# jhidalgocarrio/slam-localization

Measured on AMD Instinct MI355X. Metric: filter predict+update steps/sec, higher is better.
Workload: dtype f64

## Files before the change

slam-localization_amd/csrc/slk_kernels.hpp:

```cpp
#pragma once
#include <hip/hip_runtime.h>

#include "../../include/slk.h"
#include "slk_math.hpp"

namespace slk {

typedef double d4 __attribute__((ext_vector_type(4)));
typedef float f4 __attribute__((ext_vector_type(4)));
typedef __bf16 b8 __attribute__((ext_vector_type(8)));

constexpr int KP = 8;
constexpr int STEP_WGS = 4;
constexpr int MAXM = 32;
constexpr int PRED_SCRATCH = 1536;

struct Lay { int kind, k, nfk, nfkl, N, Nq, nso3; };

struct KArgs {
    int B;
    Lay lay;
    double *mean; double *P; int *status; unsigned *outliers;
    int do_predict, pm; const double *u; int u_stride; const double *Q; int q_stride; const double *Yext;
    int do_update, mm; const double *mp; int mp_stride; const double *z; int m;
// ... 299 lines not shown
        }
    int fail = -1;
    CholCols<NTHREADS, SD, 0>::run(a, Lp, n, colbuf, ti, tj, active, fail);
    __syncthreads();
    return (fail >= n) ? -1 : fail;
}

__host__ __device__ constexpr int tile_idx(int I, int J) { return I * (I + 1) / 2 + J; }

__device__ __forceinline__ void wave_sync() { asm volatile("s_waitcnt lgkmcnt(0)" ::: "memory"); }

template <int NT> struct CholM {
    static constexpr int NTL = NT * (NT + 1) / 2;
    static constexpr int LDC = 16 * NT + 2;
    static constexpr int COLBUF = 4 * LDC;
};

template <int NT, class InitFn>
__device__ __forceinline__ void cholm_load(d4 (&acc)[CholM<NT>::NTL], int n, int lane, InitFn init)
{
    const int c = lane & 15, g = lane >> 4;
#pragma unroll
    for (int I = 0; I < NT; ++I)
#pragma unroll
        for (int J = 0; J <= I; ++J)
#pragma unroll
            for (int r = 0; r < 4; ++r) {
                int row = 16 * I + g + 4 * r, col = 16 * J + c;
                double v;
                if (row < n && col < n) v = (row >= col) ? init(row, col) : init(col, row);
                else v = (row == col) ? 1.0 : 0.0;
                acc[tile_idx(I, J)][r] = -v;
            }
}

template <int NT, class InitFn>
__device__ __forceinline__ void cholm_load_t(d4 (&acc)[CholM<NT>::NTL], int n, int lane, InitFn init)
{
    const int c = lane & 15, g = lane >> 4;
#pragma unroll
    for (int J = 0; J < NT; ++J)
#pragma unroll
        for (int I = J; I < NT; ++I)
#pragma unroll
            for (int r = 0; r < 4; ++r) {
                int row = 16 * I + c, col = 16 * J + g + 4 * r;
                double v;
                if (row < n && col < n) v = (row >= col) ? init(row, col) : init(col, row);
                else v = (row == col) ? 1.0 : 0.0;
                acc[tile_idx(I, J)][r] = -v;
            }
}

template <int NT, class XFn, class YFn>
__device__ __forceinline__ void cholm_downdate(d4 (&acc)[CholM<NT>::NTL], int n, int kk, int lane, XFn xel, YFn yel)
{
    const int c = lane & 15, g = lane >> 4;
    for (int ks = 0; ks * 4 < kk; ++ks) {
        const int cc = 4 * ks + g;
        double af[NT], bf[NT];
#pragma unroll
        for (int I = 0; I < NT; ++I) {
            int rho = 16 * I + c;
            bool ok = cc < kk && rho < n;
            af[I] = ok ? xel(rho, cc) : 0.0;
            bf[I] = ok ? yel(rho, cc) : 0.0;
        }
#pragma unroll
        for (int I = 0; I < NT; ++I)
#pragma unroll
            for (int J = 0; J <= I; ++J)
                acc[tile_idx(I, J)] = __builtin_amdgcn_mfma_f64_16x16x4f64(af[I], bf[J], acc[tile_idx(I, J)], 0, 0, 0);
    }
}

template <int NT, int JK>
struct CholMCols {
    __device__ __forceinline__ static void run(d4 (&acc)[CholM<NT>::NTL], double *Lp, int n, double *colbuf, int lane, int &fail)
    {
        if constexpr (JK < NT) {
            constexpr int LDC = CholM<NT>::LDC;
            const int c = lane & 15, g = lane >> 4;
            if (fail < 0) {
                for (int c0 = 0; c0 < 16; c0 += 4) {
                    const int k0 = 16 * JK + c0;
                    if (k0 >= n) break;
                    if (c >= c0 && c < c0 + 4) {
                        double *dst = colbuf + (c - c0) * LDC + g;
#pragma unroll
                        for (int I = JK; I < NT; ++I)
#pragma unroll
                            for (int r = 0; r < 4; ++r) dst[16 * I + 4 * r] = acc[tile_idx(I, JK)][r];
                    }
                    wave_sync();
                    const double *pb = colbuf + k0;
                    const double p00 = -pb[0], p10 = -pb[1], p20 = -pb[2], p30 = -pb[3];
                    const double p11 = -pb[LDC + 1], p21 = -pb[LDC + 2], p31 = -pb[LDC + 3];
                    const double p22 = -pb[2 * LDC + 2], p32 = -pb[2 * LDC + 3], p33 = -pb[3 * LDC + 3];
                    double v[NT][4];
#pragma unroll
                    for (int I = JK; I < NT; ++I)
#pragma unroll
                        for (int b = 0; b < 4; ++b) v[I][b] = -colbuf[b * LDC + 16 * I + c];
                    wave_sync();
                    double s0, r0, s1, r1, s2, r2, s3, r3;
                    if (!(p00 > 0.0)) { fail = k0; break; }
// ... 5 lines not shown
                    const double l21 = fma(-l20, l10, p21) * r1, l31 = fma(-l30, l10, p31) * r1;
                    const double d2 = fma(-l21, l21, fma(-l20, l20, p22));
                    if (!(d2 > 0.0)) { fail = k0 + 2; break; }
                    rsqrt_pivot(d2, s2, r2);
                    const double l32 = fma(-l31, l21, fma(-l30, l20, p32)) * r2;
                    const double d3 = fma(-l32, l32, fma(-l31, l31, fma(-l30, l30, p33)));
                    if (!(d3 > 0.0)) { fail = k0 + 3; break; }
                    rsqrt_pivot(d3, s3, r3);
                    const int kap = k0 + g;
                    const double sg = (g == 0) ? s0 : (g == 1) ? s1 : (g == 2) ? s2 : s3;
                    double frag[NT];
#pragma unroll
                    for (int I = JK; I < NT; ++I) {
                        const double vi0 = v[I][0], vi1 = v[I][1], vi2 = v[I][2], vi3 = v[I][3];
                        const double x0 = vi0 * r0;
                        const double x1 = fma(-x0, l10, vi1) * r1;
                        const double x2 = fma(-x1, l21, fma(-x0, l20, vi2)) * r2;
                        const double x3 = fma(-x2, l32, fma(-x1, l31, fma(-x0, l30, vi3))) * r3;
                        double f = (g == 0) ? x0 : (g == 1) ? x1 : (g == 2) ? x2 : x3;
                        const int rho = 16 * I + c;
                        if (rho == kap) f = sg;
                        if (rho < kap) f = 0.0;
                        frag[I] = f;
                        if (rho >= kap && rho < n && kap < n) Lp[pk(n, rho, kap)] = f;
                    }
#pragma unroll
                    for (int J = JK; J < NT; ++J)
#pragma unroll
                        for (int I = J; I < NT; ++I)
                            acc[tile_idx(I, J)] = __builtin_amdgcn_mfma_f64_16x16x4f64(frag[I], frag[J], acc[tile_idx(I, J)], 0, 0, 0);
                }
            }
            CholMCols<NT, JK + 1>::run(acc, Lp, n, colbuf, lane, fail);
        }
    }
};

template <int NT>
__device__ __forceinline__ int cholm_factor(d4 (&acc)[CholM<NT>::NTL], double *Lp, int n, double *colbuf, int lane)
{
    int fail = -1;
    __builtin_amdgcn_s_setprio(3);
    CholMCols<NT, 0>::run(acc, Lp, n, colbuf, lane, fail);
    wave_sync();
    __builtin_amdgcn_s_setprio(0);
    return fail;
}

__device__ __forceinline__ double readlane_f64(double x, int l)
{
    return __hiloint2double(__builtin_amdgcn_readlane(__double2hiint(x), l), __builtin_amdgcn_readlane(__double2loint(x), l));
}

template <int NT, int JK, int C0, int OUT = 1>
struct CholPSteps {
    __device__ __forceinline__ static void run(d4 (&acc)[CholM<NT>::NTL], double *Lp, int n, double *colbuf, int lane, bool &bad)
    {
        if constexpr (JK < NT) {
            constexpr int LDC = CholM<NT>::LDC;
            constexpr int k0 = 16 * JK + C0;
            if (k0 < n) {
                const int c = lane & 15, g = lane >> 4;
                const int row = (NT == 4) ? lane : min(lane, 16 * NT - 1);
                auto live = [&](int p) { return OUT != 2 || k0 + p < n; };
                const bool last = OUT == 2 && k0 + 4 >= n;
#pragma unroll
                for (int I = JK; I < NT; ++I) colbuf[g * LDC + 16 * I + c] = acc[tile_idx(I, JK)][C0 / 4];
                wave_sync();
                double l[4];
#pragma unroll
                for (int p = 0; p < 4; ++p) l[p] = live(p) ? -colbuf[p * LDC + row] : 0.0;
#pragma unroll
                for (int p = 0; p < 4; ++p) {
                    if (!live(p)) continue;
                    const double d = readlane_f64(l[p], k0 + p);
                    {
                        int nb = !(d > 0.0);
                        asm volatile("" : "+v"(nb));
                        bad |= (nb != 0);
                    }
                    double sq, rs;
                    rsqrt_pivot(d, sq, rs);
                    (void)sq;
                    l[p] *= rs;
#pragma unroll
                    for (int q = p + 1; q < 4; ++q)
                        if (live(q)) l[q] = fma(-l[p], readlane_f64(l[p], k0 + q), l[q]);
                }
                if (!last) {
                    wave_sync();
                    if (NT == 4 || lane < 16 * NT) {
#pragma unroll
                        for (int p = 0; p < 4; ++p) colbuf[p * LDC + lane] = l[p];
                    }
                }
#pragma unroll
                for (int p = 0; p < 4; ++p) {
                    if constexpr (OUT == 2) {
                        if (lane >= 16 * JK && (NT == 4 || lane < 16 * NT)) {
                            const int It = lane >> 4;
                            Lp[(It * (It + 1) / 2 + JK) * 256 + (C0 + p) * 16 + (lane & 15)] = (k0 + p < n && lane >= k0 + p) ? l[p] : 0.0;
                        }
                    } else if constexpr (OUT == 1) {
                        typedef __attribute__((address_space(1))) double gdouble;
                        unsigned long long colb = reinterpret_cast<unsigned long long>(Lp + pkcol(n, k0 + p));
                        asm volatile("" : "+s"(colb));
                        gdouble *colp = reinterpret_cast<gdouble *>(colb);
                        if (k0 + p < n && lane >= k0 + p && lane < n) colp[lane] = l[p];
                    } else {
                        if (k0 + p < n && lane >= k0 + p && lane < n) Lp[pkcol(n, k0 + p) + lane] = l[p];
                    }
                }
                if (!last) {
                    constexpr int J0 = (C0 == 12) ? JK + 1 : JK;
                    wave_sync();
                    double frag[NT];
#pragma unroll
                    for (int I = J0; I < NT; ++I) frag[I] = colbuf[g * LDC + 16 * I + c];
                    wave_sync();
#pragma unroll
                    for (int J = J0; J < NT; ++J)
#pragma unroll
                        for (int I = J; I < NT; ++I)
                            acc[tile_idx(I, J)] = __builtin_amdgcn_mfma_f64_16x16x4f64(frag[J], frag[I], acc[tile_idx(I, J)], 0, 0, 0);
                }
            } else if constexpr (OUT == 2) {
                if (lane >= 16 * JK && (NT == 4 || lane < 16 * NT)) {
                    const int It = lane >> 4;
#pragma unroll
                    for (int p = 0; p < 4; ++p) Lp[(It * (It + 1) / 2 + JK) * 256 + (C0 + p) * 16 + (lane & 15)] = 0.0;
                }
            }
            CholPSteps<NT, (C0 == 12 ? JK + 1 : JK), (C0 + 4) & 15, OUT>::run(acc, Lp, n, colbuf, lane, bad);
        }
    }
};

template <int NT, int OUT = 1>
__device__ __forceinline__ int cholp_factor(d4 (&acc)[CholM<NT>::NTL], double *Lp, int n, double *colbuf, int lane)
{
    bool bad = false;
    CholPSteps<NT, 0, 0, OUT>::run(acc, Lp, n, colbuf, lane, bad);
    wave_sync();
    return bad ? 0 : -1;
}

template <int NMAX, class InitFn>
__device__ __forceinline__ int chol_rows(double *Lp, int n, int lane, InitFn init, int nst = -1)
{
    if (nst < 0) nst = n;
    static_assert(NMAX <= 32, "chol_rows keeps a row per lane in registers");
    double a[NMAX];
#pragma unroll
    for (int j = 0; j < NMAX; ++j) {
        a[j] = init(min(lane, n - 1), j < n ? j : 0);
        if ((j & 3) == 3) __builtin_amdgcn_sched_barrier(0);
    }
    bool bad = false;
#pragma unroll
    for (int j = 0; j < NMAX; ++j) {
        if (j < n) {
            const double d = readlane_f64(a[j], j);
            bad |= !(d > 0.0);
            double sq, rs;
            rsqrt_pivot(d, sq, rs);
            (void)sq;
            a[j] *= rs;
#pragma unroll
            for (int k = j + 1; k < NMAX; ++k) a[k] = fma(-a[j], readlane_f64(a[j], k), a[k]);
            __builtin_amdgcn_sched_barrier(0);
        }
    }
    if (lane < nst) {
#pragma unroll
        for (int j = 0; j < NMAX; ++j)
            if (j < nst && lane >= j) Lp[pk(nst, lane, j)] = a[j];
    }
    wave_sync();
    return bad ? 0 : -1;
}

template <int NT, class InitFn>
__device__ __forceinline__ void cholw_load(d4 (&acc)[NT], int n, int lane, int wave, InitFn init)
{
    const int c = lane & 15, g = lane >> 4;
#pragma unroll
    for (int J = 0; J < NT; ++J)
#pragma unroll
        for (int r = 0; r < 4; ++r) {
            int row = 16 * wave + g + 4 * r, col = 16 * J + c;
            double v = 0.0;
            if (J <= wave && wave < NT) {
                if (row < n && col < n) v = (row >= col) ? init(row, col) : init(col, row);
                else v = (row == col) ? 1.0 : 0.0;
            }
            acc[J][r] = -v;
        }
// ... 1043 lines not shown
                constexpr int I = TileMap<NT>::row(T), J = TileMap<NT>::col(T);
                const int c = 16 * J + (lane & 15), rc = MfmaTiles<NT, NW, 0>::rho_of(c);
#pragma unroll
                for (int r = 0; r < 4; ++r) {
                    const int rr = 16 * I + 4 * (lane >> 4) + r;
                    if (rr < N && c < N) {
                        const int r1 = MfmaTiles<NT, NW, 0>::rho_of(rr);
                        double v = (double)acc[T / NW][r];
                        if (r1 >= 0 && rc >= 0) {
                            const int hi = r1 > rc ? r1 : rc, lo = r1 > rc ? rc : r1;
                            const int ti = hi >> 4, tj = lo >> 4;
                            v += EEt[(ti * (ti + 1) / 2 + tj) * 272 + (lo & 15) * 17 + (hi & 15)];
                        }
                        gP[c + (size_t)rr * N] = v;
                        if (I != J) gP[rr + (size_t)c * N] = v;
                    }
                }
            }
            MfmaTiles32<NT, NW, T + 1>::store_plus_rot(gP, N, acc, wave, lane, EEt);
        }
    }
    __device__ __forceinline__ static void store(double *gP, int N, const f4 (&acc)[TPW], int wave, int lane, int pass)
    {
        if constexpr (T < TileMap<NT>::NTILES) {
            if ((T % NW) == wave && (T / PER_PASS) == pass) {
                constexpr int I = TileMap<NT>::row(T), J = TileMap<NT>::col(T);
                int c = 16 * J + (lane & 15);
#pragma unroll
                for (int r = 0; r < 4; ++r) {
                    int rr = 16 * I + 4 * (lane >> 4) + r;
                    if (rr < N && c < N) {
                        double v = 0.5 * (double)acc[(T % PER_PASS) / NW][r];
                        gP[c + (size_t)rr * N] = v;
                        if (I != J) gP[rr + (size_t)c * N] = v;
                    }
                }
            }
            MfmaTiles32<NT, NW, T + 1>::store(gP, N, acc, wave, lane, pass);
        }
    }
};

template <int K> __device__ __forceinline__ bool msckf_step_fast(const KArgs &a, double *smem);
template <int NT, int NTHREADS, int KST, int MST> struct HasFastStep {
    static constexpr bool value = KST >= 4 && KST <= 8 && MST == 8 && NTHREADS == 256 && NT == (12 + 6 * KST + 15) / 16;
};

template <int NT, int NTHREADS, int KST = -1, int MST = 0>
__global__ __launch_bounds__(NTHREADS, (NTHREADS >= 256 && NT >= 3 && NT <= 4 ? (MST > 0 ? STEP_WGS : 2) : ((NT >= 5 && NT <= 8) ? 2 : (NT <= 2 ? 4 : 1)))) void msckf_step_kernel(KArgs a)
{
    constexpr bool BIG = NT > 4;
    extern __shared__ __attribute__((aligned(16))) double smem[];
    if constexpr (HasFastStep<NT, NTHREADS, KST, MST>::value) {
        if (!a.do_predict && a.do_update && msckf_step_fast<KST>(a, smem)) return;
    }
    constexpr int NW = NTHREADS / 64;
    constexpr int NROWS = (NT <= 2 && KST >= 0) ? 12 + 6 * KST : 1;
    static_assert(NT > 2 || NTHREADS == 64, "states of N <= 32 run one wave per filter");
    const int bidx = blockIdx.x, tid = threadIdx.x, lane = tid & 63, wave = tid >> 6;
    Lay L = a.lay;
    L.kind = SLK_MSCKF;
    if constexpr (KST >= 0) { L.k = KST; L.N = 12 + 6 * KST; L.Nq = 13 + 7 * KST; L.nso3 = 1 + KST; }
    if constexpr (MST > 0) { a.m = MST; a.emit = 0; a.do_update = 1; if (NT <= 4) a.rebuild_prec = 0; }
    const int N = L.N, Nq = L.Nq, m = a.m, nso3 = L.nso3;
    const Carve cv = carve_step(L, m, NT, BIG, (KST >= 0 && MST > 0 && !BIG) ? 0 : a.rebuild_prec);
    const int S = cv.S, LDD = cv.LDD;
    double *Lp = BIG ? a.wsL + (size_t)bidx * pk_size(N) : smem + cv.Lp;
    double *mu = smem + cv.mu, *ref = smem + cv.ref;
    double *delta = smem + cv.delta, *md = smem + cv.md, *colbuf = smem + cv.colbuf, *pool = smem + cv.pool, *cq = smem + cv.cq;
    int *ish = reinterpret_cast<int *>(smem + cv.small);
    int *roff = ish + 48;
    double *gmean = a.mean + (size_t)bidx * Nq;
    double *gP = a.P + (size_t)bidx * N * N;
    double *omean = a.mean_out ? a.mean_out + (size_t)bidx * Nq : gmean;
    double *oP = a.P_out ? a.P_out + (size_t)bidx * N * N : gP;
    int status = 0;
    if (a.do_update && a.emit != 4 && tid == 0) a.outliers[bidx] = 0u;
    SLK_STAMP(0);

    for (int e = tid; e < Nq; e += NTHREADS) mu[e] = gmean[e];
    if (tid == 0) {
        int o = 0;
        for (int b = 0; b < nso3; ++b) { roff[b] = o; o += rot_count(L, b); }
        roff[nso3] = o;
        ish[42] = 0;
    }
    __syncthreads();
    SLK_STAMP(1);

    constexpr bool WCHOL = NT >= 3 && NT <= 4 && NW >= NT;
    bool pred12 = false;
    const double *Pn12 = smem + cv.pn12;
    if constexpr (NT <= 2) {
        if (a.do_predict) {
            double *Lblk = pool, *Pn = pool + 160, *scr = pool + 320;
            const int st = predict_phase<false>(a, bidx, tid, [&](int i, int j) { return gP[i + (size_t)j * N]; }, Lblk, mu, Pn, scr,
                                                nullptr);
            if (st < 0) return;
            status |= st;
            if (!(st & SLK_ST_LLT_FAIL)) {
                for (int e = tid; e < 144; e += NTHREADS) {
                    smem[cv.pn12 + e] = Pn[e];
                    gP[(e % 12) + (size_t)(e / 12) * N] = Pn[e];
                }
                if (tid < 13) gmean[tid] = mu[tid];
                pred12 = true;
// ... 1241 lines not shown
```

slam-localization_amd/csrc/slk_math.hpp:

```cpp
#pragma once
#include <hip/hip_runtime.h>

namespace slk {

struct Quat { double x, y, z, w; };

__device__ __forceinline__ Quat qmul(const Quat &a, const Quat &b)
{
    Quat o;
    o.w = a.w * b.w - a.x * b.x - a.y * b.y - a.z * b.z;
    o.x = a.w * b.x + a.x * b.w + a.y * b.z - a.z * b.y;
    o.y = a.w * b.y + a.y * b.w + a.z * b.x - a.x * b.z;
    o.z = a.w * b.z + a.z * b.w + a.x * b.y - a.y * b.x;
    return o;
}

__device__ __forceinline__ Quat qconj(const Quat &q) { return Quat{-q.x, -q.y, -q.z, q.w}; }

__device__ __forceinline__ void qrot(const Quat &q, double vx, double vy, double vz,
                                     double &ox, double &oy, double &oz)
{
    double ux = q.y * vz - q.z * vy, uy = q.z * vx - q.x * vz, uz = q.x * vy - q.y * vx;
    ux += ux; uy += uy; uz += uz;
    ox = vx + q.w * ux + (q.y * uz - q.z * uy);
    oy = vy + q.w * uy + (q.z * ux - q.x * uz);
    oz = vz + q.w * uz + (q.x * uy - q.y * ux);
}

struct CosSinc { double c, s; };
__device__ __forceinline__ CosSinc cos_sinc_sqrt_libm_body(double x)
{
    const double sx = sqrt(x);
    return CosSinc{cos(sx), sin(sx) / sx};
}
__device__ __forceinline__ double so3_log_scale_libm_body(double n2, double w)
{
    double nv = sqrt(n2);
    if (nv < 1e-11) nv = 1e-11;
    return 2.0 / nv * atan(nv / w);
}
__device__ __attribute__((noinline)) CosSinc cos_sinc_sqrt_libm(double x) { return cos_sinc_sqrt_libm_body(x); }
__device__ __attribute__((noinline)) double so3_log_scale_libm(double n2, double w) { return so3_log_scale_libm_body(n2, w); }

template <bool LEAF = false>
__device__ __forceinline__ void cos_sinc_sqrt(double x, double &c, double &s)
{
    if (x < 0.25) {
        const double y = -x;
        double cc = 0x1.1d8d32755f8fbp-29;
        cc = fma(cc, y, 0x1.27e40964b47d4p-22);
        cc = fma(cc, y, 0x1.a01a00fb1bc6fp-16);
        cc = fma(cc, y, 0x1.6c16c16bdd04ep-10);
        cc = fma(cc, y, 0x1.5555555555421p-5);
        cc = fma(cc, y, 0x1.fffffffffffffp-2);
        cc = fma(cc, y, 1.0);
        double ss = 0x1.ac53ce336f805p-26;
        ss = fma(ss, y, 0x1.71dd113fb7905p-19);
        ss = fma(ss, y, 0x1.a01a01061c190p-13);
        ss = fma(ss, y, 0x1.11111110ecfb3p-7);
        ss = fma(ss, y, 0x1.555555555548fp-3);
        ss = fma(ss, y, 1.0);
        c = cc;
        s = ss;
    } else {
        const CosSinc r = LEAF ? cos_sinc_sqrt_libm_body(x) : cos_sinc_sqrt_libm(x);
        c = r.c;
        s = r.s;
    }
}

template <bool LEAF = false>
__device__ __forceinline__ Quat so3_exp(double vx, double vy, double vz)
{
    double c, s;
    cos_sinc_sqrt<LEAF>(0.25 * (vx * vx + vy * vy + vz * vz), c, s);
    double m = s * 0.5;
    return Quat{m * vx, m * vy, m * vz, c};
}

__device__ __forceinline__ double rcp_refined(double a)
// ... 119 lines not shown
```

slam-localization_amd/csrc/slk_step_fast.hpp:

```cpp
#pragma once
#ifdef SLK_STAMPS
#define SLK_FSTAMP(i) do { SLK_STAMP_NR(i); if (a.stop > 0 && a.stop == (i)) return true; } while (0)
#define SLK_WSTAMP(w, i) do { if (tid == 64 * (w) && a.dbg) a.dbg[(size_t)bidx * 32 + (i)] = clock64(); } while (0)
#define SLK_FBAIL(code) do { SLK_NOTE(28, code); return false; } while (0)
#else
#define SLK_FSTAMP(i) do { } while (0)
#define SLK_WSTAMP(w, i) do { } while (0)
#define SLK_FBAIL(code) return false
#endif

namespace slk {

template <int K> struct FastShape {
    static constexpr int N = 12 + 6 * K, Nq = 13 + 7 * K, S = 2 * N + 1, NSO3 = K + 1;
    static constexpr int NT = (N + 15) / 16, NTL = NT * (NT + 1) / 2, NKS = (N + 3) / 4;
    static constexpr int NROT = 3 * NSO3;
    static constexpr int NP = 3 * K * K + 15 * K + 6;
    static constexpr int NIT = NP + NSO3;
    static constexpr int RND = (NIT + 255) / 256;
    static constexpr int oLt = 0;
    static constexpr int oMu = oLt + NTL * 256;
    static constexpr int oRef = oMu + ((Nq + 7) & ~7);
    static constexpr int oDelta = oRef + ((Nq + 7) & ~7);
    static constexpr int oMd = oDelta + 64;
// ... 150 lines not shown
        for (int i = 0; i < NV; ++i) f[i] = fma(f[i], y[i], ak);
    }
#pragma unroll
    for (int i = 0; i < NV; ++i) {
        f[i] = fma(f[i], y[i], 1.0);
        const double sv = sc[i] * f[i];
        d[i][0] = sv * q[i].x; d[i][1] = sv * q[i].y; d[i][2] = sv * q[i].z;
    }
    return true;
}

template <int E0, int CNT>
__device__ __forceinline__ void fast_scan_entries(const double (&av)[8], double (&G)[20])
{
#pragma unroll
    for (int e = 0; e < CNT; ++e) {
        constexpr int dummy = 0; (void)dummy;
        const int q = E0 + e;
        const int r = (q >= 1) + (q >= 3) + (q >= 6) + (q >= 10) + (q >= 15) + (q >= 21) + (q >= 28), cc = q - r * (r + 1) / 2;
        const double pr = av[r] * av[cc];
        G[e] = wave_inclusive_scan(pr) - pr;
    }
}

template <int K> struct FastPairTable {
    unsigned long long v[FastShape<K>::NP];
    constexpr FastPairTable() : v{}
    {
        int p = 0;
        for (int b = 0; b <= K; ++b) {
            const int to = b ? 9 + 6 * b : 3;
            for (int j = 0; j < to + 3; ++j, ++p) {
                unsigned long long a[3] = {0, 0, 0};
                for (int cc = 0; cc < 3; ++cc) {
                    const int t = to + cc, I = t >> 4, Jc = j >> 4;
                    a[cc] = (unsigned long long)(FastShape<K>::oLt + (Jc <= I ? (I * (I + 1) / 2 + Jc) * 256 + (j & 15) * 16 + (t & 15) : 16));
                }
                const int rho = 3 * b;
                const unsigned long long e0 = (unsigned long long)(((j >> 2) * 2 + (rho >> 4)) * 64 + (j & 3) * 16 + (rho & 15));
                const unsigned long long sd = (b == 1 && j >= 16) ? (unsigned long long)(j - 15) : 0ull;
                v[p] = a[0] | (a[1] << 13) | ((unsigned long long)b << 26) | (sd << 30) | (a[2] << 32) | (e0 << 45);
            }
        }
    }
};
template <int K> struct FastPairTableHolder { static __device__ const FastPairTable<K> tab; };
template <int K> __device__ const FastPairTable<K> FastPairTableHolder<K>::tab = FastPairTable<K>();

#define SLK_G(r, c) Gf[(r) * ((r) + 1) / 2 + (c)]
__device__ __forceinline__ bool fast_ldm_columns(double (&Gf)[36], const double *dZi, const double *Sm, unsigned kept, int lane, int N,
                                                 double *Wb, double *mdiag)
{
    const bool live = lane < N;
#pragma unroll
    for (int r = 0; r < 8; ++r) {
        const bool kr = (kept >> r) & 1u;
#pragma unroll
        for (int c = 0; c <= r; ++c) {
            const bool in = kr && ((kept >> c) & 1u);
            const double sv = Sm[in ? r + 8 * c : 0];
            SLK_G(r, c) = in ? sv - SLK_G(r, c) : ((r == c) ? 1.0 : 0.0);
        }
    }
    double y[8];
    bool ok = true;
#pragma unroll
    for (int j = 0; j < 8; ++j) {
        double d = SLK_G(j, j);
#pragma unroll
        for (int p = 0; p < j; ++p) d = fma(-SLK_G(j, p), SLK_G(j, p), d);
        ok = ok && (d > 0.0);
        double sq, rs;
        rsqrt_pivot(d, sq, rs);
        SLK_G(j, j) = rs;
#pragma unroll
        for (int i = j + 1; i < 8; ++i) {
            double v = SLK_G(i, j);
#pragma unroll
            for (int p = 0; p < j; ++p) v = fma(-SLK_G(i, p), SLK_G(j, p), v);
            SLK_G(i, j) = v * rs;
        }
        const double aj = dZi[(j >> 1) * 128 + 2 * lane + (j & 1)];
        double sacc = ((kept >> j) & 1u) ? 0.5 * aj : 0.0;
#pragma unroll
        for (int p = 0; p < j; ++p) sacc = fma(-SLK_G(j, p), y[p], sacc);
        y[j] = sacc * rs;
    }
    double dj = 1.0;
#pragma unroll
    for (int c = 0; c < 8; ++c) dj = fma(-y[c], y[c], dj);
    ok = ok && (dj > 0.0);
    double sqd, rsd;
    rsqrt_pivot(dj, sqd, rsd);
    const double sc = -0.5 * rsd;
#pragma unroll
    for (int c = 7; c >= 0; --c) {
        double sacc = y[c];
#pragma unroll
        for (int p = c + 1; p < 8; ++p) sacc = fma(-SLK_G(p, c), y[p], sacc);
        y[c] = sacc * SLK_G(c, c);
        Wb[bw_idx(lane, c)] = live ? y[c] * sc : 0.0;
    }
    mdiag[lane] = live ? sqd : 1.0;
    return __all(ok) != 0;
}
#undef SLK_G

template <int NT, class FillFn>
__device__ __forceinline__ void ldm_product_tiled(double *Lt, const double *dZi, const double *Wb, const double *mdiag, int lane,
                                                  int wave, int JB, FillFn fill)
{
    const int c = lane & 15, g = lane >> 4;
    const int lw = (g >> 1) * 128 + 2 * c + (g & 1);
    constexpr int MAXT = (NT == 4) ? 4 : 2;
    d4 acc[MAXT];
#pragma unroll
    for (int q = 0; q < MAXT; ++q) acc[q] = d4{0.0, 0.0, 0.0, 0.0};
#pragma unroll
    for (int I = 0; I < NT; ++I)
#pragma unroll
// ... 116 lines not shown
                                               d4 (&acc)[FastShape<K>::NT], bool lower_only)
{
    using F = FastShape<K>;
    constexpr int NT = F::NT, N = F::N, EES = FastEE<K>::EES, PAD = FastEE<K>::PAD;
    const int c = lane & 15, g = lane >> 4;
    {
        const int rj = fast_rho<N>(16 * J + c);
        const double bf = pd[g == 0 ? 32 + rj : (g == 1 ? rj : 31)];
#pragma unroll
        for (int I = J; I < NT; ++I) {
            const int ri = fast_rho<N>(16 * I + c);
            const double af = pd[g == 0 ? ri : (g == 1 ? 32 + ri : 31)];
            acc[I - J] = __builtin_amdgcn_mfma_f64_16x16x4f64(af, bf, acc[I - J], 0, 0, 0);
        }
        const double *eec = ee + (rj & PAD);
#pragma unroll
        for (int I = J; I < NT; ++I) {
            const unsigned rw = g == 0 ? fast_rho_pack<K>(I, 0) : (g == 1 ? fast_rho_pack<K>(I, 1) : (g == 2 ? fast_rho_pack<K>(I, 2) : fast_rho_pack<K>(I, 3)));
#pragma unroll
            for (int r = 0; r < 4; ++r) acc[I - J][r] += eec[((rw >> (8 * r)) & 0xffu) * EES];
        }
    }
    double *o = oP + c + g * N;
#pragma unroll
    for (int I = J; I < NT; ++I) {
#pragma unroll
        for (int r = 0; r < 4; ++r) {
            const bool full = 16 * I + 4 * r + 3 < N && 16 * J + 15 < N;
            if (I > J && lower_only) continue;
            if (16 * I + 4 * r < N && (full || (16 * I + 4 * r + g < N && 16 * J + c < N)))
                o[16 * J + (16 * I + 4 * r) * N] = acc[I - J][r];
        }
        if (I > J) {
            double *buf = bufs + (I * (I - 1) / 2 + J) * 272;
#pragma unroll
            for (int r = 0; r < 4; ++r) buf[c * 17 + g + 4 * r] = acc[I - J][r];
            wave_sync();
#pragma unroll
            for (int q = 0; q < 4; ++q) {
                const double v = buf[(g + 4 * q) * 17 + c];
                const bool full = 16 * I + 15 < N;
                if (full || 16 * I + c < N) o[16 * I + (16 * J + 4 * q) * N] = v;
            }
        }
    }
}

template <int K>
__device__ __forceinline__ bool msckf_step_fast(const KArgs &a, double *smem)
{
    using F = FastShape<K>;
    constexpr int N = F::N, Nq = F::Nq, S = F::S, NSO3 = F::NSO3, NT = F::NT, NKS = F::NKS, NROT = F::NROT;
    constexpr int NP = F::NP;
    if (a.mm != SLK_MM_FEATURE_PROJ || a.gate == 2 || a.emit != 0 || a.rebuild_prec != 0 || !a.mp || a.m != 8) return false;
    const int bidx = blockIdx.x, tid = threadIdx.x, lane = tid & 63;
    const int wave = __builtin_amdgcn_readfirstlane(tid >> 6);
    const int c16 = lane & 15, g4 = lane >> 4;
    double *Lt = smem + F::oLt, *mu = smem + F::oMu, *ref = smem + F::oRef, *delta = smem + F::oDelta, *md32 = smem + F::oMd;
    double *d0 = smem + F::oD0, *d0s = smem + F::oD0s, *pd = smem + F::oPd, *cq = smem + F::oCq, *str = smem + F::oStr, *U = smem + F::oU;
    int *ints = reinterpret_cast<int *>(smem + F::oInts);
    double *T = smem + F::oTab;
    double *Yp = U + F::uYp, *Wb = U + F::uW, *dZi = U + F::uDZ, *Sm = U + F::uSm, *mdiag = U + F::uMdiag, *bvec = U + F::uB;
    double *innov = U + F::uInnov, *dz0 = U + F::uDz0, *tmpS = U + F::uTmp, *Et = U;
    const double *gmean = a.mean + (size_t)bidx * Nq;
    const double *gP = a.P + (size_t)bidx * N * N;
    const double *mp = a.mp + (size_t)bidx * a.mp_stride;
    SLK_STAMP_NR(0);

    int jmax = 0, bad;
    const bool here = a.wsfail == nullptr;
    {
        const double *gL = here ? gP : a.wsL + (size_t)bidx * pk_size(N);
        const int t = lane, It = t >> 4;
        const int lbase = (It * (It + 1) / 2) * 256 + wave * 16 + (t & 15);
        double v[16];
        if (!here) {
#pragma unroll
            for (int u = 0; u < 16; ++u) {
                const int j = 4 * u + wave;
                const bool in = j < N && t >= j && t < N;
                v[u] = gL[in ? pkcol(N, j) + t : 0];
            }
        }
        const double mu0 = (tid < Nq) ? gmean[tid] : 0.0;
        const int t0 = (tid && tid < NSO3) ? 9 + 6 * tid : 3;
        const double pdg = gP[t0 * (N + 1)] + gP[(t0 + 1) * (N + 1)] + gP[(t0 + 2) * (N + 1)];
        const double tabv = fast_series_table[tid < 26 ? tid : 25];
        bad = here ? 0 : (a.wsfail[bidx] >= 0);
        bool ok = true;
#pragma unroll
        for (int f = 0; f < 4; ++f) {
            const double cf = mp[4 * f + 3];
            ok = ok && (cf >= 0.0) && (cf <= (double)K);
            const int cp = ok ? (int)cf : 0, tp = cp ? 6 + 6 * cp : 0;
            jmax = (tp + 5 > jmax) ? tp + 5 : jmax;
        }
        bad |= !ok;
        if (tid < NSO3) bad |= !(pdg < 9.869604401089358);
        if (tid < Nq) mu[tid] = mu0;
        if (tid < 64) { str[tid] = 0.0; pd[tid] = 0.0; ints[tid] = 0; }
        if (tid < 32) { d0[tid] = 0.0; md32[tid] = 0.0; }
        if (tid < 26) T[tid] = tabv;
        if (!here) {
#pragma unroll
            for (int u = 0; u < 16; ++u) {
                const int j = 4 * u + wave;
                const bool in = j < N && t >= j && t < N;
                if ((u >> 2) < NT && It >= (u >> 2) && It < NT) Lt[lbase + (u >> 2) * 256 + (u & 3) * 64] = in ? v[u] : 0.0;
            }
        }
        if (here && wave == 0) {
            d4 fa[CholM<NT>::NTL];
            cholm_load_t<NT>(fa, N, lane, [&](int i, int j) { return gP[i + (size_t)j * N]; });
            bad |= cholp_factor<NT, 2>(fa, Lt, N, U, lane) >= 0;
        }
    }
    if (__syncthreads_or(bad)) SLK_FBAIL(2);
    SLK_FSTAMP(3);

    {
        const int f = wave;
        const int cp = (int)mp[4 * f + 3];
        const int tp = cp ? 6 + 6 * cp : 0, sp = cp ? 6 + 7 * cp : 0;
        const double fx = mp[4 * f], fy = mp[4 * f + 1], fz = mp[4 * f + 2];
        const int j = lane, Jc = j >> 4;
        const bool act = j < tp + 6;
        double l[6], x[7];
#pragma unroll
        for (int q = 0; q < 6; ++q) {
            const int t = tp + q, I = t >> 4;
            const bool in = act && Jc <= I;
            l[q] = Lt[in ? (I * (I + 1) / 2 + Jc) * 256 + (j & 15) * 16 + (t & 15) : 16];
        }
#pragma unroll
        for (int q = 0; q < 7; ++q) x[q] = mu[sp + q];
        double zp0, zp1, zm0, zm1;
        {
            const double rv[2][3] = {{l[3], l[4], l[5]}, {-l[3], -l[4], -l[5]}};
            Quat ex[2];
            if (!__all(so3_exp_tab<2>(T, rv, ex))) ints[50] = 1;
            const Quat qx = Quat{x[3], x[4], x[5], x[6]};
            double lx, ly, lz;
            auto quot = [](double lx_, double ly_, double lz_, double &q0, double &q1) __attribute__((always_inline)) {
                const double r = rcp_refined(lz_);
                q0 = lx_ * r; q0 = fma(fma(-lz_, q0, lx_), r, q0);
                q1 = ly_ * r; q1 = fma(fma(-lz_, q1, ly_), r, q1);
            };
            qrot(qconj(qmul(qx, ex[0])), fx - (x[0] + l[0]), fy - (x[1] + l[1]), fz - (x[2] + l[2]), lx, ly, lz);
            quot(lx, ly, lz, zp0, zp1);
            qrot(qconj(qmul(qx, ex[1])), fx - (x[0] - l[0]), fy - (x[1] - l[1]), fz - (x[2] - l[2]), lx, ly, lz);
            quot(lx, ly, lz, zm0, zm1);
        }
        const double Z00 = readlane_f64(zp0, 63), Z01 = readlane_f64(zp1, 63);
        const double yp0 = zp0 - Z00, yp1 = zp1 - Z01, ym0 = zm0 - Z00, ym1 = zm1 - Z01;
        Yp[j * 17 + 2 * f] = yp0; Yp[j * 17 + 2 * f + 1] = yp1;
        Yp[j * 17 + 8 + 2 * f] = ym0; Yp[j * 17 + 8 + 2 * f + 1] = ym1;
        dZi[f * 128 + 2 * j] = yp0 - ym0; dZi[f * 128 + 2 * j + 1] = yp1 - ym1;
        const double s0 = wave_sum_f64(yp0 + ym0), s1 = wave_sum_f64(yp1 + ym1);
        if (lane == 0) {
            const double e0 = s0 * (1.0 / (double)S), e1 = s1 * (1.0 / (double)S);
            innov[2 * f] = a.z[(size_t)bidx * 8 + 2 * f] - (Z00 + e0);
            innov[2 * f + 1] = a.z[(size_t)bidx * 8 + 2 * f + 1] - (Z01 + e1);
            dz0[2 * f] = e0; dz0[2 * f + 1] = e1;
        }
    }
    __syncthreads();
    if (ints[50]) SLK_FBAIL(3);
// ... 20 lines not shown
        if (wave == 2) fast_scan_entries<0, 16>(av, Gs);
        else fast_scan_entries<16, 20>(av, Gs);
        SLK_WSTAMP(3, 21);
    }
    __syncthreads();
    SLK_FSTAMP(6);

    unsigned kept = 0xffu, nout = 0u;
    if (a.gate) {
        const int p = 2 * (lane & 3), q = p + 1;
        const double s00 = Sm[p + 8 * p], s01 = Sm[p + 8 * q], s10 = Sm[q + 8 * p], s11 = Sm[q + 8 * q];
        const double det = s00 * s11 - s01 * s10, r0 = innov[p], r1 = innov[q];
        const double d2 = (r0 * (s11 * r0 - s01 * r1) + r1 * (s00 * r1 - s10 * r0)) / det;
        if (!__all(d2 < 5.99)) {
            int *ix = ints + 10 * wave;
            if (lane == 0) {
                int cnt = 8, i = 0;
                unsigned no = 0;
                for (int r = 0; r < 8; ++r) ix[r] = r;
                while (i < cnt / 2) {
                    const int pp = ix[2 * i], qq = ix[2 * i + 1];
                    const double t00 = Sm[pp + 8 * pp], t01 = Sm[pp + 8 * qq], t10 = Sm[qq + 8 * pp], t11 = Sm[qq + 8 * qq];
                    const double dt = t00 * t11 - t01 * t10, u0 = innov[pp], u1 = innov[qq];
                    const double dd = (u0 * (t11 * u0 - t01 * u1) + u1 * (t00 * u1 - t10 * u0)) / dt;
                    if (!(dd < 5.99)) {
                        for (int rep = 0; rep < 2; ++rep) {
                            const int pos = 2 * i + rep, numRows = cnt - 1;
                            if (pos < numRows) for (int w = pos; w < numRows; ++w) ix[w] = ix[w + 1];
                            cnt = numRows;
                        }
                        no++;
                    } else {
                        i++;
                    }
                }
                unsigned kp = 0;
                for (int r = 0; r < cnt; ++r) kp |= 1u << ix[r];
                ix[8] = (int)kp; ix[9] = (int)no;
            }
            wave_sync();
            kept = (unsigned)ix[8]; nout = (unsigned)ix[9];
        }
    }
    if (kept == 0u) SLK_FBAIL(4);
    SLK_FSTAMP(7);

    if (wave == 2) {
#pragma unroll
        for (int e = 0; e < 16; ++e) Yp[e * 64 + lane] = Gs[e];
    }
    __syncthreads();
    if (wave == 0) {
        double gg[8][8], gi[8], y[8];
#pragma unroll
        for (int i = 0; i < 8; ++i)
#pragma unroll
            for (int j = 0; j <= i; ++j) {
                const bool in = ((kept >> i) & 1u) && ((kept >> j) & 1u);
                const double v = Sm[in ? i + 8 * j : 0];
                gg[i][j] = in ? v : (i == j ? 1.0 : 0.0);
            }
        bool spd = true;
#pragma unroll
        for (int j = 0; j < 8; ++j) {
            double d = gg[j][j];
#pragma unroll
            for (int p = 0; p < j; ++p) d = fma(-gg[j][p], gg[j][p], d);
            spd = spd && (d > 0.0);
            double sq, rs;
            rsqrt_pivot(d, sq, rs);
            gi[j] = rs;
#pragma unroll
            for (int i = j + 1; i < 8; ++i) {
                double v = gg[i][j];
#pragma unroll
                for (int p = 0; p < j; ++p) v = fma(-gg[i][p], gg[j][p], v);
                gg[i][j] = v * rs;
            }
            double s = ((kept >> j) & 1u) ? innov[j] : 0.0;
#pragma unroll
            for (int p = 0; p < j; ++p) s = fma(-gg[j][p], y[p], s);
            y[j] = s * rs;
        }
#pragma unroll
        for (int cc = 7; cc >= 0; --cc) {
            double s = y[cc];
#pragma unroll
            for (int p = cc + 1; p < 8; ++p) s = fma(-gg[p][cc], y[p], s);
            y[cc] = s * gi[cc];
        }
        if (!spd && lane == 0) ints[49] = 1;
        SLK_WSTAMP(0, 24);
        double bj = 0.0;
#pragma unroll
        for (int cc = 0; cc < 8; ++cc) bj = fma(dZi[(cc >> 1) * 128 + 2 * lane + (cc & 1)], y[cc], bj);
        bvec[lane] = 0.5 * bj;
        wave_sync();
        {
            const int t = lane, It = t >> 4;
            const double *Lrow = Lt + (It * (It + 1) / 2) * 256 + (t & 15);
            double part[NT];
#pragma unroll
            for (int Jb = 0; Jb < NT; ++Jb) {
                double s = 0.0;
#pragma unroll
                for (int jj = 0; jj < 16; ++jj) {
                    if (16 * Jb + jj < N) s = fma(Lrow[Jb * 256 + jj * 16], bvec[16 * Jb + jj], s);
                    if ((jj & 7) == 7) __builtin_amdgcn_sched_barrier(0);
                }
                part[Jb] = s;
            }
            double dl = part[0];
#pragma unroll
            for (int Jb = 1; Jb < NT; ++Jb) dl += (It >= Jb) ? part[Jb] : 0.0;
// ... 236 lines not shown
```

Baseline: 23.64 million.

## Specialize tile Cholesky for compile-time N with exact loads and LDS stores

Adds a compile-time-N loader that reads the covariance into MFMA tiles using one scalar base per tile column and immediate offsets. The tile Cholesky variant now writes its columns into LDS through exec-masked ds_write sequences and reads its update fragments back from that buffer, instead of staging through colbuf with extra barriers. The zero fill of the tile buffer moves to the other three waves and is followed by a block barrier. The pivot check becomes a scalar rank test. The 8x8 Gram load and its Cholesky get a fast path for when all eight measurements are kept. These changes target memory latency, barriers and predicate work in the update step, at the cost of inline assembly and tighter shape assumptions.

```diff
diff --git a/slam-localization_amd/csrc/slk_kernels.hpp b/slam-localization_amd/csrc/slk_kernels.hpp
--- a/slam-localization_amd/csrc/slk_kernels.hpp
+++ b/slam-localization_amd/csrc/slk_kernels.hpp
@@ -375,6 +375,53 @@
             }
 }
 
+template <int NT, int N>
+__device__ __forceinline__ void cholm_load_t_exact(d4 (&acc)[CholM<NT>::NTL], const double *gP, int lane)
+{
+    static_assert(N > 16 * (NT - 1) && N <= 16 * NT, "N fills NT tile rows");
+    constexpr int RL = N - 16 * (NT - 1);
+    constexpr bool PADDED = RL < 16;
+    constexpr long MID = 2560;
+    static_assert(8L * (12 * N + 16 * (NT - 1) + 16) - MID < 4096 && MID <= 4096, "one base per tile column");
+    const int c = lane & 15, g = lane >> 4;
+    const unsigned below = 8u * (unsigned)(c + g * N);
+    const bool rowin = !PADDED || c < RL;
+    unsigned diag[4], diagl[4];
+    bool din[4];
+#pragma unroll
+    for (int r = 0; r < 4; ++r) {
+        const int cc = g + 4 * r, hi = c > cc ? c : cc, lo = c > cc ? cc : c;
+        diag[r] = 8u * (unsigned)(hi + lo * N);
+        din[r] = !PADDED || hi < RL;
+        diagl[r] = din[r] ? diag[r] : 0u;
+    }
+#pragma unroll
+    for (int J = 0; J < NT; ++J) {
+        typedef __attribute__((address_space(1))) const char gchar;
+        typedef __attribute__((address_space(1))) const double gcdouble;
+        unsigned long long pin = reinterpret_cast<unsigned long long>(gP) + (8L * 16 * J * N + MID);
+        asm volatile("" : "+s"(pin));
+        gchar *sb = reinterpret_cast<gchar *>(pin);
+#pragma unroll
+        for (int I = J; I < NT; ++I)
+#pragma unroll
+            for (int r = 0; r < 4; ++r) {
+                const bool lastrow = PADDED && I == NT - 1;
+                double v;
+                if (I == J) {
+                    gchar *lp = sb + (lastrow ? diagl[r] : diag[r]);
+                    v = *reinterpret_cast<gcdouble *>(lp + (8L * 16 * J - MID));
+                    if (lastrow) v = din[r] ? v : (c == g + 4 * r ? 1.0 : 0.0);
+                } else {
+                    gchar *lp = sb + (lastrow && !rowin ? 0u : below);
+                    v = *reinterpret_cast<gcdouble *>(lp + (8L * (16 * I + 4 * r * N) - MID));
+                    if (lastrow) v = rowin ? v : 0.0;
+                }
+                acc[tile_idx(I, J)][r] = -v;
+            }
+    }
+}
+
 template <int NT, class XFn, class YFn>
 __device__ __forceinline__ void cholm_downdate(d4 (&acc)[CholM<NT>::NTL], int n, int kk, int lane, XFn xel, YFn yel)
 {
@@ -486,13 +533,35 @@
     return __hiloint2double(__builtin_amdgcn_readlane(__double2hiint(x), l), __builtin_amdgcn_readlane(__double2loint(x), l));
 }
 
-template <int NT, int JK, int C0, int OUT = 1>
+template <int LO, int HI, int OFF>
+__device__ __forceinline__ void lds_store4_lane_ranges(unsigned addr, const double (&v)[4])
+{
+    constexpr int W0 = HI - LO > 0 ? HI - LO : 0, W1 = HI - LO - 1 > 0 ? HI - LO - 1 : 0;
+    constexpr int W2 = HI - LO - 2 > 0 ? HI - LO - 2 : 0, W3 = HI - LO - 3 > 0 ? HI - LO - 3 : 0;
+    static_assert(LO >= 0 && HI <= 64 && W0 < 64 && LO + 3 < 64 && OFF >= 0 && OFF + 384 < 65536, "s_bfm_b64 fields, ds offset");
+    unsigned long long save;
+    asm volatile("s_mov_b64 %[sv], exec\n\t"
+                 "s_bfm_b64 exec, %[w0], %[l0]\n\tds_write_b64 %[a], %[v0] offset:%[o0]\n\t"
+                 "s_bfm_b64 exec, %[w1], %[l1]\n\tds_write_b64 %[a], %[v1] offset:%[o1]\n\t"
+                 "s_bfm_b64 exec, %[w2], %[l2]\n\tds_write_b64 %[a], %[v2] offset:%[o2]\n\t"
+                 "s_bfm_b64 exec, %[w3], %[l3]\n\tds_write_b64 %[a], %[v3] offset:%[o3]\n\t"
+                 "s_mov_b64 exec, %[sv]"
+                 : [sv] "=&s"(save)
+                 : [a] "v"(addr), [v0] "v"(v[0]), [v1] "v"(v[1]), [v2] "v"(v[2]), [v3] "v"(v[3]),
+                   [w0] "n"(W0), [w1] "n"(W1), [w2] "n"(W2), [w3] "n"(W3), [l0] "n"(LO), [l1] "n"(LO + 1), [l2] "n"(LO + 2), [l3] "n"(LO + 3),
+                   [o0] "n"(OFF), [o1] "n"(OFF + 128), [o2] "n"(OFF + 256), [o3] "n"(OFF + 384)
+                 : "memory");
+}
+
+template <int NT, int JK, int C0, int OUT = 1, int NC = 0>
 struct CholPSteps {
-    __device__ __forceinline__ static void run(d4 (&acc)[CholM<NT>::NTL], double *Lp, int n, double *colbuf, int lane, bool &bad)
+    __device__ __forceinline__ static void run(d4 (&acc)[CholM<NT>::NTL], double *Lp, int n, double *colbuf, int lane, unsigned &bad)
     {
+        static_assert(OUT != 2 || (NC > 0 && NC <= 16 * NT), "the tile variant takes n as a template argument too");
         if constexpr (JK < NT) {
             constexpr int LDC = CholM<NT>::LDC;
             constexpr int k0 = 16 * JK + C0;
+            if constexpr (OUT == 2) n = NC;
             if (k0 < n) {
                 const int c = lane & 15, g = lane >> 4;
                 const int row = (NT == 4) ? lane : min(lane, 16 * NT - 1);
@@ -501,47 +570,55 @@
 #pragma unroll
                 for (int I = JK; I < NT; ++I) colbuf[g * LDC + 16 * I + c] = acc[tile_idx(I, JK)][C0 / 4];
                 wave_sync();
-                double l[4];
-#pragma unroll
-                for (int p = 0; p < 4; ++p) l[p] = live(p) ? -colbuf[p * LDC + row] : 0.0;
+                double m[4], l[4];
+#pragma unroll
+                for (int p = 0; p < 4; ++p) m[p] = live(p) ? colbuf[p * LDC + row] : 0.0;
 #pragma unroll
                 for (int p = 0; p < 4; ++p) {
+                    l[p] = 0.0;
                     if (!live(p)) continue;
-                    const double d = readlane_f64(l[p], k0 + p);
+                    const double mpiv = readlane_f64(m[p], k0 + p), d = -mpiv;
                     {
-                        int nb = !(d > 0.0);
-                        asm volatile("" : "+v"(nb));
-                        bad |= (nb != 0);
+                        if constexpr (OUT == 2) {
+                            const unsigned rk = pivot_rank_neg((unsigned)__double2hiint(mpiv), (unsigned)__double2loint(mpiv));
+                            bad = rk > bad ? rk : bad;
+                            asm volatile("" : "+s"(bad));
+                        } else {
+                            int nb = !(d > 0.0);
+                            asm volatile("" : "+v"(nb));
+                            bad |= (nb != 0) ? 0x7ff00000u : 0u;
+                        }
                     }
                     double sq, rs;
                     rsqrt_pivot(d, sq, rs);
                     (void)sq;
-                    l[p] *= rs;
+                    l[p] = m[p] * -rs;
 #pragma unroll
                     for (int q = p + 1; q < 4; ++q)
-                        if (live(q)) l[q] = fma(-l[p], readlane_f64(l[p], k0 + q), l[q]);
-                }
-                if (!last) {
+                        if (live(q)) m[q] = fma(l[p], readlane_f64(l[p], k0 + q), m[q]);
+                }
+                if constexpr (OUT != 2) {
                     wave_sync();
                     if (NT == 4 || lane < 16 * NT) {
 #pragma unroll
                         for (int p = 0; p < 4; ++p) colbuf[p * LDC + lane] = l[p];
                     }
                 }
+                if constexpr (OUT == 2) {
+                    typedef __attribute__((address_space(3))) double ldouble;
+                    const int It = lane >> 4;
+                    const unsigned trow = (unsigned)(size_t)(ldouble *)Lp + (It * (It + 1) / 2 * 256 + (lane & 15)) * 8;
+                    lds_store4_lane_ranges<k0, NC, (JK * 256 + C0 * 16) * 8>(trow, l);
+                }
 #pragma unroll
                 for (int p = 0; p < 4; ++p) {
-                    if constexpr (OUT == 2) {
-                        if (lane >= 16 * JK && (NT == 4 || lane < 16 * NT)) {
-                            const int It = lane >> 4;
-                            Lp[(It * (It + 1) / 2 + JK) * 256 + (C0 + p) * 16 + (lane & 15)] = (k0 + p < n && lane >= k0 + p) ? l[p] : 0.0;
-                        }
-                    } else if constexpr (OUT == 1) {
+                    if constexpr (OUT == 1) {
                         typedef __attribute__((address_space(1))) double gdouble;
                         unsigned long long colb = reinterpret_cast<unsigned long long>(Lp + pkcol(n, k0 + p));
                         asm volatile("" : "+s"(colb));
                         gdouble *colp = reinterpret_cast<gdouble *>(colb);
                         if (k0 + p < n && lane >= k0 + p && lane < n) colp[lane] = l[p];
-                    } else {
+                    } else if constexpr (OUT == 0) {
                         if (k0 + p < n && lane >= k0 + p && lane < n) Lp[pkcol(n, k0 + p) + lane] = l[p];
                     }
                 }
@@ -549,34 +626,33 @@
                     constexpr int J0 = (C0 == 12) ? JK + 1 : JK;
                     wave_sync();
                     double frag[NT];
-#pragma unroll
-                    for (int I = J0; I < NT; ++I) frag[I] = colbuf[g * LDC + 16 * I + c];
-                    wave_sync();
+                    if constexpr (OUT == 2) {
+#pragma unroll
+                        for (int I = J0; I < NT; ++I) frag[I] = Lp[tile_idx(I, JK) * 256 + (C0 + g) * 16 + c];
+                    } else {
+#pragma unroll
+                        for (int I = J0; I < NT; ++I) frag[I] = colbuf[g * LDC + 16 * I + c];
+                        wave_sync();
+                    }
 #pragma unroll
                     for (int J = J0; J < NT; ++J)
 #pragma unroll
                         for (int I = J; I < NT; ++I)
                             acc[tile_idx(I, J)] = __builtin_amdgcn_mfma_f64_16x16x4f64(frag[J], frag[I], acc[tile_idx(I, J)], 0, 0, 0);
                 }
-            } else if constexpr (OUT == 2) {
-                if (lane >= 16 * JK && (NT == 4 || lane < 16 * NT)) {
-                    const int It = lane >> 4;
-#pragma unroll
-                    for (int p = 0; p < 4; ++p) Lp[(It * (It + 1) / 2 + JK) * 256 + (C0 + p) * 16 + (lane & 15)] = 0.0;
-                }
-            }
-            CholPSteps<NT, (C0 == 12 ? JK + 1 : JK), (C0 + 4) & 15, OUT>::run(acc, Lp, n, colbuf, lane, bad);
+            }
+            CholPSteps<NT, (C0 == 12 ? JK + 1 : JK), (C0 + 4) & 15, OUT, NC>::run(acc, Lp, n, colbuf, lane, bad);
         }
     }
 };
 
-template <int NT, int OUT = 1>
+template <int NT, int OUT = 1, int NC = 0>
 __device__ __forceinline__ int cholp_factor(d4 (&acc)[CholM<NT>::NTL], double *Lp, int n, double *colbuf, int lane)
 {
-    bool bad = false;
-    CholPSteps<NT, 0, 0, OUT>::run(acc, Lp, n, colbuf, lane, bad);
+    unsigned bad = 0u;
+    CholPSteps<NT, 0, 0, OUT, NC>::run(acc, Lp, n, colbuf, lane, bad);
     wave_sync();
-    return bad ? 0 : -1;
+    return pivot_rank_not_positive(bad) ? 0 : -1;
 }
 
 template <int NMAX, class InitFn>
@@ -1726,6 +1802,7 @@
     constexpr bool BIG = NT > 4;
     extern __shared__ __attribute__((aligned(16))) double smem[];
     if constexpr (HasFastStep<NT, NTHREADS, KST, MST>::value) {
+        static_assert(NTHREADS == 256, "msckf_step_fast is written for four waves (its tile fill, its wave roles)");
         if (!a.do_predict && a.do_update && msckf_step_fast<KST>(a, smem)) return;
     }
     constexpr int NW = NTHREADS / 64;
diff --git a/slam-localization_amd/csrc/slk_math.hpp b/slam-localization_amd/csrc/slk_math.hpp
--- a/slam-localization_amd/csrc/slk_math.hpp
+++ b/slam-localization_amd/csrc/slk_math.hpp
@@ -26,6 +26,19 @@
     oy = vy + q.w * uy + (q.z * ux - q.x * uz);
     oz = vz + q.w * uz + (q.x * uy - q.y * ux);
 }
+
+__host__ __device__ __forceinline__ unsigned pivot_rank_neg(unsigned xhi, unsigned xlo)
+{
+#if defined(__HIP_DEVICE_COMPILE__)
+    unsigned rk;
+    asm("s_cmp_lg_u32 %2, 0\n\ts_addc_u32 %0, %1, 0x7fffffff" : "=s"(rk) : "s"(xhi), "s"(xlo) : "scc");
+    return rk;
+#else
+    return xhi + 0x7fffffffu + (xlo != 0u ? 1u : 0u);
+#endif
+}
+__host__ __device__ __forceinline__ bool pivot_rank_not_positive(unsigned rank) { return rank >= 0x7ff00000u; }
+__host__ __device__ __forceinline__ bool pivot_not_positive(unsigned hi, unsigned lo) { return pivot_rank_not_positive(pivot_rank_neg(hi ^ 0x80000000u, lo)); }
 
 struct CosSinc { double c, s; };
 __device__ __forceinline__ CosSinc cos_sinc_sqrt_libm_body(double x)
diff --git a/slam-localization_amd/csrc/slk_step_fast.hpp b/slam-localization_amd/csrc/slk_step_fast.hpp
--- a/slam-localization_amd/csrc/slk_step_fast.hpp
+++ b/slam-localization_amd/csrc/slk_step_fast.hpp
@@ -226,20 +226,23 @@
                                                  double *Wb, double *mdiag)
 {
     const bool live = lane < N;
-#pragma unroll
-    for (int r = 0; r < 8; ++r) {
-        const bool kr = (kept >> r) & 1u;
-#pragma unroll
-        for (int c = 0; c <= r; ++c) {
-            const bool in = kr && ((kept >> c) & 1u);
-            const double sv = Sm[in ? r + 8 * c : 0];
-            SLK_G(r, c) = in ? sv - SLK_G(r, c) : ((r == c) ? 1.0 : 0.0);
-        }
-    }
+    const bool full = kept == 0xffu;
     double y[8];
     bool ok = true;
 #pragma unroll
     for (int j = 0; j < 8; ++j) {
+        if (full) {
+#pragma unroll
+            for (int r = j; r < 8; ++r) SLK_G(r, j) = Sm[r + 8 * j] - SLK_G(r, j);
+        } else {
+            const bool kj = (kept >> j) & 1u;
+#pragma unroll
+            for (int r = j; r < 8; ++r) {
+                const bool in = kj && ((kept >> r) & 1u);
+                const double sv = Sm[in ? r + 8 * j : 0];
+                SLK_G(r, j) = in ? sv - SLK_G(r, j) : ((r == j) ? 1.0 : 0.0);
+            }
+        }
         double d = SLK_G(j, j);
 #pragma unroll
         for (int p = 0; p < j; ++p) d = fma(-SLK_G(j, p), SLK_G(j, p), d);
@@ -462,6 +465,7 @@
     using F = FastShape<K>;
     constexpr int N = F::N, Nq = F::Nq, S = F::S, NSO3 = F::NSO3, NT = F::NT, NKS = F::NKS, NROT = F::NROT;
     constexpr int NP = F::NP;
+    constexpr int NTHREADS = 256;
     if (a.mm != SLK_MM_FEATURE_PROJ || a.gate == 2 || a.emit != 0 || a.rebuild_prec != 0 || !a.mp || a.m != 8) return false;
     const int bidx = blockIdx.x, tid = threadIdx.x, lane = tid & 63;
     const int wave = __builtin_amdgcn_readfirstlane(tid >> 6);
@@ -519,10 +523,15 @@
                 if ((u >> 2) < NT && It >= (u >> 2) && It < NT) Lt[lbase + (u >> 2) * 256 + (u & 3) * 64] = in ? v[u] : 0.0;
             }
         }
-        if (here && wave == 0) {
+        if (here) {
             d4 fa[CholM<NT>::NTL];
-            cholm_load_t<NT>(fa, N, lane, [&](int i, int j) { return gP[i + (size_t)j * N]; });
-            bad |= cholp_factor<NT, 2>(fa, Lt, N, U, lane) >= 0;
+            if (wave == 0) cholm_load_t_exact<NT, N>(fa, gP, lane);
+            else {
+                double2 *Lt2 = reinterpret_cast<double2 *>(Lt);
+                for (int e = tid - 64; e < CholM<NT>::NTL * 128; e += NTHREADS - 64) Lt2[e] = double2{0.0, 0.0};
+            }
+            __syncthreads();
+            if (wave == 0) bad |= cholp_factor<NT, 2, N>(fa, Lt, N, U, lane) >= 0;
         }
     }
     if (__syncthreads_or(bad)) SLK_FBAIL(2);
@@ -649,14 +658,23 @@
     __syncthreads();
     if (wave == 0) {
         double gg[8][8], gi[8], y[8];
-#pragma unroll
-        for (int i = 0; i < 8; ++i)
-#pragma unroll
-            for (int j = 0; j <= i; ++j) {
-                const bool in = ((kept >> i) & 1u) && ((kept >> j) & 1u);
-                const double v = Sm[in ? i + 8 * j : 0];
-                gg[i][j] = in ? v : (i == j ? 1.0 : 0.0);
-            }
+        if (kept == 0xffu) {
+#pragma unroll
+            for (int i = 0; i < 8; ++i) {
+#pragma unroll
+                for (int j = 0; j <= i; ++j) gg[i][j] = Sm[i + 8 * j];
+            }
+        } else {
+#pragma unroll
+            for (int i = 0; i < 8; ++i) {
+#pragma unroll
+                for (int j = 0; j <= i; ++j) {
+                    const bool in = ((kept >> i) & 1u) && ((kept >> j) & 1u);
+                    const double v = Sm[in ? i + 8 * j : 0];
+                    gg[i][j] = in ? v : (i == j ? 1.0 : 0.0);
+                }
+            }
+        }
         bool spd = true;
 #pragma unroll
         for (int j = 0; j < 8; ++j) {
```

After: 24.16 million (median of 6 runs). 2.2% higher.
